# lgw-frank/Short_LDPC_Decoding_OSD

Measured on AMD Instinct MI355X. Metric: decoded frames/sec + FER, (128,64) LDPC NMS-10+OSD-2 @ 2.5 dB, higher is better.
Workload: dtype f32; 1 GPU; nms10_osd2 -- configs[3]: NMS-10 + OSD-2, 2^20 frames over 8 GPUs = 131 072 per GPU; code=CCSDS (128,64), osd_order=2, frames_per_gpu=131072, parallelism=frame-sharded x1, rccl_ranks=1, distinct_batches_per_gpu=4, distinct_frames=524288, bytes_in_plus_out_per_rotation=545783808, nms_kernel=qc16, streams=1, osd_route=front+search

## Files before the change

### short_ldpc_decoding_osd_amd/csrc/ldpc_front.h

```cpp
#pragma once
#include "ldpc_internal.h"
#include "ldpc_wave.h"

namespace ldpc {

struct __attribute__((aligned(16))) FrontLds {
    RankLds rank;
    u64 colbuf[64];
    unsigned mask[4];
    unsigned char pi1[128];
    unsigned char rowsrc[64];
    unsigned char perm[128];
};

struct FrontResult {
    int o1, o2;
    u64 Prow;
    int ns;
};


template <bool GE_LANE_OPAQUE = false>
__device__ __forceinline__ FrontResult front_device_vals(FrontLds &L, unsigned a1, unsigned a2, const u64 *__restrict__ Gcols, int lane)
{
    const float bs = bucket_scale(a1, a2);
    int r1, r2;
    bucket_ranks(L.rank, ((u64)a1 << 32) | (unsigned)(127 - lane), ((u64)a2 << 32) | (unsigned)(63 - lane), bucket_of(a1, bs),
                 bucket_of(a2, bs), lane, r1, r2);
    L.pi1[r1] = (unsigned char)lane;
    L.pi1[r2] = (unsigned char)(lane + 64);
    if (lane < 4) L.mask[lane] = 0;
    wave_fence();
    u64 C1 = Gcols[L.pi1[lane]];
    u64 C2 = Gcols[L.pi1[lane + 64]];
    int rho = lane, idx1 = lane, idx2 = lane + 64;
    int ge_lane = lane;
    if constexpr (GE_LANE_OPAQUE) asm volatile("" : "+v"(ge_lane));
    const int ns = ge_columns(C1, C2, rho, idx1, idx2, ge_lane, nullptr);
    int rankM = lane, rankL = lane;
    if (ns != 0) {
        atomicOr(&L.mask[idx1 >> 5], 1u << (idx1 & 31));
        wave_fence();
        const unsigned m[4] = {L.mask[0], L.mask[1], L.mask[2], L.mask[3]};
        rankM = below_mask(m, idx1);
        rankL = idx2 - below_mask(m, idx2);
    }
    L.perm[rankM] = L.pi1[idx1];
    L.perm[64 + rankL] = L.pi1[idx2];
    L.colbuf[rankL] = C2;
    L.rowsrc[rankM] = (unsigned char)rho;
    wave_fence();
    const u64 R = transpose64(L.colbuf[lane], lane);
    FrontResult res;
    res.Prow = shfl64(R, L.rowsrc[lane]);
    res.o1 = L.perm[lane];
    res.o2 = L.perm[64 + lane];
    res.ns = ns;
    wave_fence();
    return res;
}

template <bool GE_LANE_OPAQUE = false>
__device__ __forceinline__ FrontResult front_device(FrontLds &L, const float *__restrict__ y, long long src,
                                                    const u64 *__restrict__ Gcols, int lane)
{
    return front_device_vals<GE_LANE_OPAQUE>(L, __float_as_uint(y[src * 128 + lane]) & 0x7FFFFFFFu, __float_as_uint(y[src * 128 + 64 + lane]) & 0x7FFFFFFFu, Gcols, lane);
}


}
```

### short_ldpc_decoding_osd_amd/csrc/ldpc_internal.h

```cpp
#pragma once

#include <hip/hip_runtime.h>
#include <stdint.h>

#include <initializer_list>
#include <mutex>
#include <string>
#include <unordered_map>
#include <vector>

#include "../../include/ldpc_osd.h"
#include "ldpc_osd_tables.h"

namespace ldpc {

int fail(int code, const char *fmt, ...) __attribute__((format(printf, 2, 3)));
int hip_fail(hipError_t e, const char *what);

struct NamedPtr {
    const char *name;
    const void *ptr;
};
inline int first_null(const char *who, std::initializer_list<NamedPtr> required)
{
    for (const NamedPtr &r : required)
        if (!r.ptr) return fail(LDPC_E_ARG, "%s: %s is NULL", who, r.name);
    return LDPC_OK;
}

#define LDPC_HIP(call)                                      \
    do {                                                    \
        hipError_t e__ = (call);                            \
        if (e__ != hipSuccess) return ::ldpc::hip_fail(e__, #call); \
    } while (0)

inline unsigned frame_grid(int64_t F) { return (unsigned)(F < 65536 ? F : 65536); }

constexpr int kMaxIters = 64;

struct AlphaArg {
    float a[kMaxIters];
};

struct QcTerm {
    int br, bc, s;
};

}

struct ldpc_code {
    int n = 0, m = 0, k = 0, max_chk_degree = 0, max_var_degree = 0, E = 0;
    std::vector<int32_t> H;
    std::vector<int32_t> G;
    std::vector<int32_t> chk_ptr;
    std::vector<int32_t> chk_var;
    std::vector<int32_t> var_ptr;
    std::vector<int32_t> var_edge;
    bool qc16_ccsds = false;
};

struct ldpc_ctx {
    int device = 0, cu_count = 256;
    ldpc_code code;
    int32_t *d_chk_ptr = nullptr, *d_chk_var = nullptr, *d_var_ptr = nullptr, *d_var_edge = nullptr;
    ldpc::OsdTables osd_tables;
    ldpc::OsdwTables osdw_tables;
    uint64_t *d_Hcols = nullptr;
    uint32_t *d_gen_G = nullptr;
    uint64_t *d_HcolsW = nullptr;
    bool dpp_ror_up = true;
    int dpp_wave_rol_dir = 0;
    bool osd_ok = false;
    bool hosd_ok = false;
    bool hosdx_ok = false;
    bool hosdw_ok = false;
    void *osd_state = nullptr;
    hipEvent_t *timing = nullptr;
    unsigned timing_recorded[LDPC_TIMING_SLOTS] = {};
};

namespace ldpc {

int gf2elim(int32_t *M, int m, int n, std::vector<int32_t> *swaps);
int build_code(ldpc_code &c);
int64_t tep_table(int k, int order, uint8_t *supports, int64_t *boundaries);
int64_t tep_table_fs(int k, int w, uint8_t *supports);
int64_t hosd_pattern_teps(int nseg, const int32_t *bounds, const int32_t *pattern, uint8_t *teps);

int launch_nms(ldpc_ctx *ctx, const float *d_llr, int64_t B, int T, const float *alpha, float w_in, float w_out,
               float *d_soft, float *d_traj, uint64_t *d_hard, uint8_t *d_fail, int kernel, hipStream_t st,
               const int32_t *d_index = nullptr, const int32_t *d_count = nullptr, float *d_rows = nullptr);
int probe_dpp(bool *ror_up, int *wave_rol_dir);
int launch_nms_train(ldpc_ctx *ctx, const float *d_llr, const uint64_t *d_label, int64_t B, int T, const float *alpha,
                     float w_in, float w_out, float *d_loss, float *d_grad, double *d_loss_sum, double *d_grad_sum,
                     float *d_traj, uint64_t *d_hard, uint8_t *d_fail, hipStream_t st);
int check_params(ldpc_ctx *ctx, const ldpc_osd_params *p, bool front_outside, const char *who);
enum class OsdRoute {
    Fused2r,
    Search2r,
    Search2,
    Table,
    Fs,
    PbStaged,
    PbFrontInside,
};
struct OsdPlan {
    OsdRoute route;
    int pb_mode;
};
OsdPlan select_route(const ldpc_ctx *ctx, const ldpc_osd_params *p, bool front_outside);
int osd_launch(ldpc_ctx *ctx, const float *d_y, const int32_t *d_index, const int32_t *d_count, int64_t F, const uint8_t *d_perm,
               const uint64_t *d_parity, const ldpc_osd_params *p, uint64_t *d_cw, float *d_metric, int32_t *d_best, int32_t *d_ntep,
               const uint64_t *d_label, int64_t *d_counts, hipStream_t s, bool *counted);
int eval_and_compact(ldpc_ctx *ctx, const uint64_t *d_hard, const uint64_t *d_label, const uint8_t *d_fail, int64_t B,
                     int64_t *d_counts, int32_t *d_index, int32_t *d_count, hipStream_t st);
int gen_ctx_init(ldpc_ctx *ctx);
void gen_ctx_release(ldpc_ctx *ctx);
int launch_gen(ldpc_ctx *ctx, const ldpc_gen_params *p, int64_t B, float *d_y, uint64_t *d_label_bits, hipStream_t st);

}
```

### short_ldpc_decoding_osd_amd/csrc/ldpc_osd.hip

```cpp
#include <math.h>
#include <stdlib.h>

#include "ldpc_osd_small.h"
#include "ldpc_osd_scan2.h"
#include "ldpc_osd_scan2r.h"
#include "ldpc_osd_fs.h"
#include "ldpc_osd_aux.h"
#include "ldpc_osd_state.h"

namespace ldpc {

int osd_ctx_init(ldpc_ctx *ctx)
{
    const OsdTables &t = ctx->osd_tables;
    ctx->osd_ok = false;
    if (t.n != kOsdN || t.k != kOsdK) return LDPC_OK;
    OsdState *st = new OsdState();
    ctx->osd_state = st;
    {
        int base2[127];
        auto npairs = [](int t) { return (t - 1) / 2 - (t > 63 ? t - 63 : 0) + 1; };
        for (int sidx = 0; sidx < 127; ++sidx) {
            int acc = 0;
            for (int t = sidx + 1; t <= 125; ++t) acc += npairs(t);
            base2[sidx] = acc;
        }
        LDPC_HIP(hipMalloc((void **)&st->d_base2, sizeof(base2)));
        LDPC_HIP(hipMemcpy(st->d_base2, base2, sizeof(base2), hipMemcpyHostToDevice));
    }
    {
        double coef[64], cdf[65], t = 0.5;
        for (int i = 0; i < 64; ++i) coef[i] = (double)(64 - i) / (double)(i + 1);
        for (int q = 0; q < 6; ++q) t = t * t;
        double acc = t;
        cdf[0] = acc;
        for (int i = 0; i < 64; ++i) { t = t * coef[i] * (0.5 / 0.5); acc = acc + t; cdf[i + 1] = acc; }
        LDPC_HIP(hipMalloc((void **)&st->d_cdf_half, sizeof(cdf)));
        LDPC_HIP(hipMemcpy(st->d_cdf_half, cdf, sizeof(cdf), hipMemcpyHostToDevice));
    }
    LDPC_HIP(hipMalloc((void **)&st->d_index_errors, sizeof(unsigned long long)));
    LDPC_HIP(hipMemset(st->d_index_errors, 0, sizeof(unsigned long long)));
    if (int rc = pb_ctx_init(ctx)) return rc;
    ctx->osd_ok = true;
    return LDPC_OK;
}

static void free_stream_ws(StreamWs &w)
{
    (void)hipFree(w.d_perm); (void)hipFree(w.d_parity); (void)hipFree(w.d_index_safe);
    (void)hipFree(w.d_pb_ctl); (void)hipFree(w.d_pb_list); (void)hipFree(w.d_pb_spill); (void)hipFree(w.d_pb_prep);
    (void)hipFree(w.d_pb_carry);
    w = StreamWs();
}

void osd_ctx_release(ldpc_ctx *ctx)
{
    if (OsdState *st = state(ctx)) {
        for (auto &kv : st->ws) free_stream_ws(kv.second);
        (void)hipFree(st->d_base2);
        (void)hipFree(st->d_cdf_half);
        (void)hipFree(st->d_index_errors);
        delete st;
    }
    ctx->osd_state = nullptr;
}

bool stream_capturing(hipStream_t s)
{
    hipStreamCaptureStatus cs = hipStreamCaptureStatusNone;
    return hipStreamIsCapturing(s, &cs) == hipSuccess && cs != hipStreamCaptureStatusNone;
}

static int stream_ws(ldpc_ctx *ctx, hipStream_t s, int64_t frames, StreamWs **out)
{
    OsdState *st = state(ctx);
    std::lock_guard<std::mutex> lock(st->mu);
    StreamWs &w = st->ws[s];
    if (frames > 0 && frames < st->reserve_frames) frames = st->reserve_frames;
    const bool capturing = stream_capturing(s);
    if (frames > w.cap) {
        if (capturing)
            return fail(LDPC_E_NOMEM, "OSD workspace of this stream holds %lld frames, %lld needed: run one call (or "
                        "ldpc_osd_reserve_stream) on the stream before capturing", (long long)w.cap, (long long)frames);
        if (w.captured)
            return fail(LDPC_E_NOMEM, "OSD workspace of this stream (%lld frames) is referenced by a captured graph and cannot grow to "
                        "%lld: destroy the graph and call ldpc_osd_release_stream, or reserve the larger size before capturing",
                        (long long)w.cap, (long long)frames);
        (void)hipFree(w.d_perm); (void)hipFree(w.d_parity);
        w.d_perm = nullptr; w.d_parity = nullptr; w.cap = 0;
        if (hipMalloc((void **)&w.d_perm, (size_t)frames * 128) != hipSuccess ||
            hipMalloc((void **)&w.d_parity, (size_t)frames * 64 * sizeof(u64)) != hipSuccess)
            return fail(LDPC_E_NOMEM, "OSD workspace for %lld frames could not be allocated", (long long)frames);
        w.cap = frames;
    }
    if (capturing) w.captured = true;
    *out = &w;
    return LDPC_OK;
}
static int guarded_index(ldpc_ctx *ctx, const ldpc_osd_params *p, const int32_t *d_index, const int32_t *d_count, int64_t F, hipStream_t s,
                         const int32_t **out)
{
    *out = d_index;
    if (!d_index || p->y_frames <= 0 || F <= 0) return LDPC_OK;
    OsdState *st = state(ctx);
    int *safe;
    {
        std::lock_guard<std::mutex> lock(st->mu);
        StreamWs &w = st->ws[s];
        if (F > w.index_cap) {
            if (stream_capturing(s) || w.captured)
                return fail(LDPC_E_NOMEM, "ldpc_osd_params.y_frames: the checked frame list of this stream holds %lld entries, %lld needed; "
                            "it cannot grow during or after a capture", (long long)w.index_cap, (long long)F);
            (void)hipFree(w.d_index_safe); w.d_index_safe = nullptr; w.index_cap = 0;
            if (hipMalloc((void **)&w.d_index_safe, sizeof(int) * (size_t)F) != hipSuccess)
                return fail(LDPC_E_NOMEM, "checked frame list for %lld frames could not be allocated", (long long)F);
            w.index_cap = F;
        }
        if (stream_capturing(s)) w.captured = true;
        safe = w.d_index_safe;
    }
    const int64_t g = (F + 255) / 256;
    hipLaunchKernelGGL(index_guard_kernel, dim3((unsigned)(g < 1024 ? g : 1024)), dim3(256), 0, s, d_index, d_count, (long long)F,
                       (long long)p->y_frames, safe, st->d_index_errors);
    LDPC_HIP(hipGetLastError());
    *out = safe;
    return LDPC_OK;
}

static unsigned osd_grid(int64_t F)
{
    const int64_t want = (F + 3) / 4;
    return (unsigned)(want < 1 ? 1 : (want < 4096 ? want : 4096));
}


static unsigned grid2r(const ldpc_ctx *ctx, int64_t F) { const int64_t g = (int64_t)ctx->cu_count * 16 * 6; return (unsigned)(F < g ? F : g); }

static void launch_front(ldpc_ctx *ctx, const float *d_y, const int32_t *d_index, const int32_t *d_count, int64_t F, uint8_t *d_perm,
                         u64 *d_parity, int32_t *d_nswaps, hipStream_t s)
{
    hipLaunchKernelGGL(osd_front_kernel, dim3(frame_grid(F)), dim3(64), 0, s, d_y, d_index, d_count, (long long)F,
                       ctx->osd_tables.d_Gcols, d_perm, d_parity, d_nswaps);
}

static int need_osd(const ldpc_ctx *ctx)
{
    return ctx->osd_ok ? LDPC_OK : fail(LDPC_E_UNSUPPORTED, "OSD kernels need an (n=128, k=64) code; this one is (%d,%d)", ctx->code.n, ctx->code.k);
}

static const char *flag_name(unsigned f)
{
    if (f & LDPC_OSD_F_TABLE_SCAN) return "LDPC_OSD_F_TABLE_SCAN";
    if (f & LDPC_OSD_F_PB_BLOCK) return "LDPC_OSD_F_PB_BLOCK";
    if (f & LDPC_OSD_F_PB_REPLAY) return "LDPC_OSD_F_PB_REPLAY";
    if (f & LDPC_OSD_F_READLANE_SCAN) return "LDPC_OSD_F_READLANE_SCAN";
    return "LDPC_OSD_F_PB_FRONT_INSIDE";
}

int check_params(ldpc_ctx *ctx, const ldpc_osd_params *p, bool front_outside, const char *who)
{
    if (int rc = need_osd(ctx)) return rc;
    if (p->order < 0 || p->order > 3) return fail(LDPC_E_ARG, "%s: order %d outside 0..3", who, p->order);
    if (p->algo != LDPC_OSD_CONVENTIONAL && p->algo != LDPC_OSD_FS && p->algo != LDPC_OSD_PB)
        return fail(LDPC_E_ARG, "%s: unknown search algorithm %d", who, p->algo);
    if (p->algo == LDPC_OSD_PB && p->order < 1) return fail(LDPC_E_ARG, "%s: PB-OSD needs order >= 1", who);
    const unsigned f = (unsigned)p->flags;
    const unsigned conv = LDPC_OSD_F_TABLE_SCAN | LDPC_OSD_F_READLANE_SCAN;
    const unsigned pb = LDPC_OSD_F_PB_BLOCK | LDPC_OSD_F_PB_REPLAY | LDPC_OSD_F_PB_FRONT_INSIDE;
    if (f & ~(conv | pb)) return fail(LDPC_E_ARG, "%s: flags 0x%x are no LDPC_OSD_F_* flag", who, f & ~(conv | pb));
    if ((f & conv) && p->algo != LDPC_OSD_CONVENTIONAL)
        return fail(LDPC_E_ARG, "%s: %s needs the conventional algorithm, not %d", who, flag_name(f & conv), p->algo);
    if ((f & LDPC_OSD_F_READLANE_SCAN) && (p->order != 2 || (f & LDPC_OSD_F_TABLE_SCAN)))
        return fail(LDPC_E_ARG, "%s: LDPC_OSD_F_READLANE_SCAN needs order 2 (not %d) and no LDPC_OSD_F_TABLE_SCAN", who, p->order);
    if ((f & pb) && p->algo != LDPC_OSD_PB)
        return fail(LDPC_E_ARG, "%s: %s needs the PB algorithm, not %d", who, flag_name(f & pb), p->algo);
    if ((f & LDPC_OSD_F_PB_REPLAY) && (f & (LDPC_OSD_F_PB_BLOCK | LDPC_OSD_F_PB_FRONT_INSIDE)))
        return fail(LDPC_E_ARG, "%s: LDPC_OSD_F_PB_REPLAY excludes %s", who, flag_name(f & (LDPC_OSD_F_PB_BLOCK | LDPC_OSD_F_PB_FRONT_INSIDE)));
    if ((f & LDPC_OSD_F_PB_FRONT_INSIDE) && front_outside)
        return fail(LDPC_E_ARG, "%s: LDPC_OSD_F_PB_FRONT_INSIDE keeps the front-end results inside the PB kernels, and this call "
                    "supplies or wants them", who);
    return LDPC_OK;
}

OsdPlan select_route(const ldpc_ctx *ctx, const ldpc_osd_params *p, bool front_outside)
{
    const unsigned f = (unsigned)p->flags;
    if (p->algo == LDPC_OSD_FS) return {OsdRoute::Fs, 0};
    if (p->algo == LDPC_OSD_PB)
        return {(f & LDPC_OSD_F_PB_FRONT_INSIDE) ? OsdRoute::PbFrontInside : OsdRoute::PbStaged,
                (f & LDPC_OSD_F_PB_REPLAY) ? 2 : ((f & LDPC_OSD_F_PB_BLOCK) ? 1 : 0)};
    if (p->order != 2 || (f & LDPC_OSD_F_TABLE_SCAN)) return {OsdRoute::Table, 0};
    if ((f & LDPC_OSD_F_READLANE_SCAN) || ctx->dpp_wave_rol_dir == 0) return {OsdRoute::Search2, 0};
    return {front_outside ? OsdRoute::Search2r : OsdRoute::Fused2r, 0};
}

int osd_launch(ldpc_ctx *ctx, const float *d_y, const int32_t *d_index, const int32_t *d_count, int64_t F, const uint8_t *d_perm,
               const uint64_t *d_parity, const ldpc_osd_params *p, uint64_t *d_cw, float *d_metric, int32_t *d_best, int32_t *d_ntep,
               const uint64_t *d_label, int64_t *d_counts, hipStream_t s, bool *counted)
{
    *counted = false;
    const OsdPlan r = select_route(ctx, p, d_perm != nullptr);
    OsdState *st = state(ctx);
    const OsdTables &t = ctx->osd_tables;
    int rc;
    if ((rc = guarded_index(ctx, p, d_index, d_count, F, s, &d_index))) return rc;
    if (!d_perm && r.route != OsdRoute::Fused2r && r.route != OsdRoute::PbFrontInside) {
        StreamWs *w;
        if ((rc = stream_ws(ctx, s, F, &w))) return rc;
        launch_front(ctx, d_y, d_index, d_count, F, w->d_perm, w->d_parity, nullptr, s);
        d_perm = w->d_perm; d_parity = reinterpret_cast<const uint64_t *>(w->d_parity);
    }
    const u64 *const parity = reinterpret_cast<const u64 *>(d_parity);
    u64 *const cw = reinterpret_cast<u64 *>(d_cw);
    const u64 *const label = d_label && d_counts ? reinterpret_cast<const u64 *>(d_label) : nullptr;
    u64 *const counts = label ? reinterpret_cast<u64 *>(d_counts) : nullptr;
    const unsigned g2r = grid2r(ctx, F), g64 = frame_grid(F);
    switch (r.route) {
    case OsdRoute::Fused2r: {
        const auto kernel = ctx->dpp_wave_rol_dir > 0 ? osd_fused2r_kernel<1> : osd_fused2r_kernel<-1>;
        hipLaunchKernelGGL(kernel, dim3(g2r), dim3(64), 0, s, d_y, d_index, d_count, (long long)F, t.d_Gcols, st->d_base2, cw, d_metric,
                           d_best, d_ntep, label, counts);
        *counted = label != nullptr;
        break;
    }
    case OsdRoute::Search2r: {
        const auto kernel = ctx->dpp_wave_rol_dir > 0 ? osd_search2r_kernel<1> : osd_search2r_kernel<-1>;
        hipLaunchKernelGGL(kernel, dim3(g2r), dim3(64), 0, s, d_y, d_index, d_count, (long long)F, d_perm, parity, st->d_base2, cw, d_metric,
                           d_best, d_ntep, label, counts);
        *counted = label != nullptr;
        break;
    }
    case OsdRoute::Search2:
        hipLaunchKernelGGL(osd_search2_kernel, dim3(g64), dim3(64), 0, s, d_y, d_index, d_count, (long long)F, d_perm, parity, st->d_base2,
                           cw, d_metric, d_best, d_ntep);
        break;
    case OsdRoute::Table:
        if (p->order >= 2)
            hipLaunchKernelGGL(osd_search_kernel<1>, dim3(g64), dim3(64), 0, s, d_y, d_index, d_count, (long long)F, d_perm, parity,
                               t.d_tep, (int)t.ntep[p->order], cw, d_metric, d_best, d_ntep);
        else
            hipLaunchKernelGGL(osd_search_kernel<4>, dim3(osd_grid(F)), dim3(256), 0, s, d_y, d_index, d_count, (long long)F, d_perm, parity,
                               t.d_tep, (int)t.ntep[p->order], cw, d_metric, d_best, d_ntep);
        break;
    case OsdRoute::Fs:
        hipLaunchKernelGGL(osd_fs_kernel, dim3(g64), dim3(64), 0, s, d_y, d_index, d_count, (long long)F, d_perm, parity, t.d_tep_fs,
                           fs_params(p, t.n, t.k, t.fs_off, t.fs_cnt), cw, d_metric, d_best, d_ntep);
        break;
    case OsdRoute::PbStaged:
        return launch_pb(ctx, d_y, d_index, d_count, F, d_perm, parity, p, r.pb_mode, false, d_cw, d_metric, d_best, d_ntep, s);
    case OsdRoute::PbFrontInside:
        return launch_pb(ctx, d_y, d_index, d_count, F, nullptr, nullptr, p, r.pb_mode, true, d_cw, d_metric, d_best, d_ntep, s);
    }
    LDPC_HIP(hipGetLastError());
    return LDPC_OK;
}

FsParams fs_params(const ldpc_osd_params *p, int n, int k, const int (&fs_off)[4], const int (&fs_cnt)[4])
{
    FsParams fp;
    fp.order = p->order; fp.quirk = p->fs_reference_quirk != 0;
    fp.beta_term = (float)((double)p->fs_beta * (double)(n - k));
    fp.tau_e = p->fs_tau_e; fp.tau_psc = p->fs_tau_psc;
    for (int w = 0; w < 4; ++w) { fp.cls_off[w] = fs_off[w]; fp.cls_cnt[w] = fs_cnt[w]; }
    return fp;
}

}

using namespace ldpc;

extern "C" {

int ldpc_osd_reserve(ldpc_ctx *ctx, int64_t max_frames)
{
    if (!ctx || max_frames < 0) return fail(LDPC_E_ARG, "ldpc_osd_reserve: bad arguments");
    if (int rc = need_osd(ctx)) return rc;
    {
        OsdState *st = state(ctx);
        std::lock_guard<std::mutex> lock(st->mu);
        if (max_frames > st->reserve_frames) st->reserve_frames = max_frames;
    }
    StreamWs *w;
    return stream_ws(ctx, nullptr, max_frames, &w);
}

int ldpc_osd_reserve_stream(ldpc_ctx *ctx, int64_t max_frames, const ldpc_osd_params *params, void *stream)
{
    if (!ctx || max_frames < 0) return fail(LDPC_E_ARG, "ldpc_osd_reserve_stream: bad arguments");
    int rc;
    if ((rc = need_osd(ctx))) return rc;
    if (params && (rc = check_params(ctx, params, false, "ldpc_osd_reserve_stream"))) return rc;
    StreamWs *w;
    if ((rc = stream_ws(ctx, (hipStream_t)stream, max_frames, &w)) || !params) return rc;
    if (params->algo == LDPC_OSD_PB && max_frames > 0) return pb_reserve(ctx, (hipStream_t)stream, max_frames, params->order);
    return LDPC_OK;
}

int ldpc_osd_release_stream(ldpc_ctx *ctx, void *stream)
{
    if (!ctx) return fail(LDPC_E_ARG, "ldpc_osd_release_stream: null ctx");
    OsdState *st = state(ctx);
    if (!st) return LDPC_OK;
    if (stream_capturing((hipStream_t)stream)) return fail(LDPC_E_ARG, "ldpc_osd_release_stream: the stream is capturing");
    std::lock_guard<std::mutex> lock(st->mu);
    auto it = st->ws.find((hipStream_t)stream);
    if (it != st->ws.end()) { free_stream_ws(it->second); st->ws.erase(it); }
    return LDPC_OK;
}

int ldpc_osd_ge(ldpc_ctx *ctx, const uint64_t *d_rows_in, int64_t F, uint64_t *d_rows_out, uint8_t *d_swaps,
                int32_t *d_nswaps, void *stream)
{
    if (!ctx || F < 0 || (F > 0 && (!d_rows_in || !d_rows_out))) return fail(LDPC_E_ARG, "ldpc_osd_ge: bad arguments");
    if (int rc = need_osd(ctx)) return rc;
    if (F == 0) return LDPC_OK;
    hipLaunchKernelGGL(osd_ge_kernel, dim3(osd_grid(F)), dim3(256), 0, (hipStream_t)stream,
                       reinterpret_cast<const u64 *>(d_rows_in), (long long)F, reinterpret_cast<u64 *>(d_rows_out), d_swaps,
                       d_nswaps);
    LDPC_HIP(hipGetLastError());
    return LDPC_OK;
}

int ldpc_osd_front(ldpc_ctx *ctx, const float *d_y, const int32_t *d_index, const int32_t *d_count, int64_t F,
                   uint8_t *d_perm, uint64_t *d_parity, int32_t *d_nswaps, void *stream)
{
    if (!ctx || F < 0 || (F > 0 && (!d_y || !d_perm || !d_parity))) return fail(LDPC_E_ARG, "ldpc_osd_front: bad arguments");
    if (int rc = need_osd(ctx)) return rc;
    if (F == 0) return LDPC_OK;
    launch_front(ctx, d_y, d_index, d_count, F, d_perm, reinterpret_cast<u64 *>(d_parity), d_nswaps, (hipStream_t)stream);
    LDPC_HIP(hipGetLastError());
    return LDPC_OK;
}

int ldpc_osd_search(ldpc_ctx *ctx, const float *d_y, const int32_t *d_index, const int32_t *d_count, int64_t F,
                    const uint8_t *d_perm, const uint64_t *d_parity, const ldpc_osd_params *p, uint64_t *d_cw,
                    float *d_metric, int32_t *d_best, int32_t *d_ntep, void *stream)
{
    if (!ctx || !p || F < 0 || (F > 0 && (!d_y || !d_cw || !d_perm || !d_parity)))
        return fail(LDPC_E_ARG, "ldpc_osd_search: bad arguments");
    int rc = check_params(ctx, p, true, "ldpc_osd_search");
    if (rc || F == 0) return rc;
    bool counted;
    return osd_launch(ctx, d_y, d_index, d_count, F, d_perm, d_parity, p, d_cw, d_metric, d_best, d_ntep, nullptr, nullptr,
                      (hipStream_t)stream, &counted);
}

int ldpc_osd_decode(ldpc_ctx *ctx, const float *d_y, const int32_t *d_index, const int32_t *d_count, int64_t F,
                    const ldpc_osd_params *p, uint64_t *d_cw, float *d_metric, int32_t *d_best, int32_t *d_ntep,
                    void *stream)
{
    if (!ctx || !p || F < 0 || (F > 0 && (!d_y || !d_cw))) return fail(LDPC_E_ARG, "ldpc_osd_decode: bad arguments");
    int rc = check_params(ctx, p, false, "ldpc_osd_decode");
    if (rc || F == 0) return rc;
    bool counted;
    return osd_launch(ctx, d_y, d_index, d_count, F, nullptr, nullptr, p, d_cw, d_metric, d_best, d_ntep, nullptr, nullptr,
                      (hipStream_t)stream, &counted);
}

int ldpc_osd_index_errors(ldpc_ctx *ctx, int64_t *count)
{
    if (!ctx || !count) return fail(LDPC_E_ARG, "ldpc_osd_index_errors: null argument");
    *count = 0;
    OsdState *st = state(ctx);
    if (!st || !st->d_index_errors) return LDPC_OK;
    unsigned long long v = 0;
    LDPC_HIP(hipMemcpy(&v, st->d_index_errors, sizeof(v), hipMemcpyDeviceToHost));
    *count = (int64_t)v;
    return LDPC_OK;
}

int ldpc_osd_tep_eval(ldpc_ctx *ctx, const float *d_y, const int32_t *d_index, const int32_t *d_count, int64_t F,
                      const uint8_t *d_perm, const uint64_t *d_parity, const uint64_t *d_mask, uint64_t *d_cw, float *d_metric,
                      int32_t *d_hd, void *stream)
{
    if (!ctx || F < 0 || (F > 0 && (!d_y || !d_perm || !d_parity || !d_mask || !d_cw)))
        return fail(LDPC_E_ARG, "ldpc_osd_tep_eval: bad arguments");
    if (int rc = need_osd(ctx)) return rc;
    if (F == 0) return LDPC_OK;
    hipLaunchKernelGGL(osd_tep_eval_kernel, dim3(osd_grid(F)), dim3(256), 0, (hipStream_t)stream, d_y, d_index, d_count, (long long)F,
                       d_perm, reinterpret_cast<const u64 *>(d_parity), reinterpret_cast<const u64 *>(d_mask),
                       reinterpret_cast<u64 *>(d_cw), d_metric, d_hd);
    LDPC_HIP(hipGetLastError());
    return LDPC_OK;
}

int ldpc_osd_counts(ldpc_ctx *ctx, const uint64_t *d_cw, const uint64_t *d_label_bits, const int32_t *d_index,
                    const int32_t *d_count, const int32_t *d_ntep, int64_t F, int64_t *d_counts, void *stream)
{
    if (!ctx || F < 0 || !d_counts || (F > 0 && (!d_cw || !d_label_bits))) return fail(LDPC_E_ARG, "ldpc_osd_counts: bad arguments");
    if (F == 0) return LDPC_OK;
    int64_t g = (F + 1023) / 1024;
    hipLaunchKernelGGL(osd_counts_kernel, dim3((unsigned)(g < 128 ? g : 128)), dim3(256), 0, (hipStream_t)stream,
                       reinterpret_cast<const u64 *>(d_cw), reinterpret_cast<const u64 *>(d_label_bits), d_index, d_count,
                       d_ntep, (long long)F, reinterpret_cast<u64 *>(d_counts));
    LDPC_HIP(hipGetLastError());
    return LDPC_OK;
}

}
```

### short_ldpc_decoding_osd_amd/csrc/ldpc_osd_small.h

```cpp
#pragma once

#include "ldpc_search.h"
#include "ldpc_front.h"

namespace ldpc {

__global__ __launch_bounds__(256) void osd_ge_kernel(const u64 *__restrict__ rows_in, long long F, u64 *__restrict__ rows_out,
        unsigned char *__restrict__ swaps, int *__restrict__ nswaps)
{
    const int lane = threadIdx.x & 63;
    const long long wave = (long long)blockIdx.x * 4 + (threadIdx.x >> 6);
    for (long long f = wave; f < F; f += (long long)gridDim.x * 4) {
        const u64 *src = rows_in + f * 128;
        u64 C1 = transpose64(src[lane * 2], lane);
        u64 C2 = transpose64(src[lane * 2 + 1], lane);
        int rho = lane, idx1 = lane, idx2 = lane + 64;
        const int ns = ge_columns(C1, C2, rho, idx1, idx2, lane, swaps ? swaps + f * 128 : nullptr);
        const u64 R1 = transpose64(C1, lane), R2 = transpose64(C2, lane);
        rows_out[f * 128 + lane * 2] = shfl64(R1, rho);
        rows_out[f * 128 + lane * 2 + 1] = shfl64(R2, rho);
        if (nswaps && lane == 0) nswaps[f] = ns;
    }
}

__global__ __launch_bounds__(64) void osd_front_kernel(const float *__restrict__ y, const int *__restrict__ index, const int *__restrict__ count,
        long long F, const u64 *__restrict__ Gcols, unsigned char *__restrict__ perm_out, u64 *__restrict__ parity_out, int *__restrict__ nswaps)
{
    __shared__ FrontLds L;
    const int lane = threadIdx.x;
    const long long nframes = frame_count(count, F);

    for (long long f = blockIdx.x; f < nframes; f += gridDim.x) {
        const long long src = index ? index[f] : f;
        const FrontResult res = front_device<true>(L, y, src, Gcols, lane);
        perm_out[f * 128 + lane] = (unsigned char)res.o1;
        perm_out[f * 128 + 64 + lane] = (unsigned char)res.o2;
        parity_out[f * 64 + lane] = res.Prow;
        if (nswaps && lane == 0) nswaps[f] = res.ns;
    }
}

template <int WAVES>
__global__ __launch_bounds__(64 * WAVES) void osd_search_kernel(const float *__restrict__ y, const int *__restrict__ index,
        const int *__restrict__ count, long long F, const unsigned char *__restrict__ perm_in, const u64 *__restrict__ parity_in,
        const uchar4 *__restrict__ teps, int ntep, u64 *__restrict__ cw_out, float *__restrict__ metric_out, int *__restrict__ best_out,
        int *__restrict__ ntep_out)
{
    __shared__ SearchLds lds[WAVES];
    const int lane = threadIdx.x & 63;
    SearchLds &L = lds[WAVES == 1 ? 0 : threadIdx.x >> 6];
    const long long nframes = frame_count(count, F);
    const long long wave = (long long)blockIdx.x * WAVES + (threadIdx.x >> 6);

    for (long long f = wave; f < nframes; f += (long long)gridDim.x * WAVES) {
        const long long src = index ? index[f] : f;
        const SearchFrame S = search_prepare(L, y, src, perm_in, parity_in, f, lane);
        float best = __builtin_inff();
        int bestt = 0x7FFFFFFF;
        u64 bestD = 0, bestE = 0;
        float bound = __builtin_inff();
        int trip = 0;
        for (int t0 = 0; t0 < ntep; t0 += 64, ++trip) {
            const int t = t0 + lane;
            if (t < ntep) {
                u64 D, E;
                float mrb, c;
                tep_apply(L, teps[t], S.d0, D, E, mrb);
                if (tep_cost_bounded(L, mrb, D, bound, c) && c < best) { best = c; bestt = t; bestD = D; bestE = E; }
            }
            if ((trip & 7) == 0) bound = wave_min_f32(best);
        }
        wave_argmin(best, bestt, bestD, bestE, lane);
        search_finish(L, S, bestE, bestD, f, lane, cw_out);
        store_results(f, lane, best, bestt, ntep, metric_out, best_out, ntep_out);
    }
}

}
```

Measured before the change: 582.4 million frames/s.

## Prefetch next frame's LLRs and indices, stage Gcols in LDS, shrink front grid

The OSD front kernel now software-pipelines its frame loop. It loads the next frame's received values and the index two frames ahead while the current frame's Gaussian elimination runs, which hides global-load latency. The generator columns are copied once per block into shared memory, so the permuted gathers read LDS instead of global memory. The grid is capped at cu_count*32 blocks so each block loops over several frames and the prefetch has work to overlap. This costs extra registers and LDS per block, and fewer blocks may lower occupancy when the frame count is small.

```diff
diff --git a/short_ldpc_decoding_osd_amd/csrc/ldpc_front.h b/short_ldpc_decoding_osd_amd/csrc/ldpc_front.h
--- a/short_ldpc_decoding_osd_amd/csrc/ldpc_front.h
+++ b/short_ldpc_decoding_osd_amd/csrc/ldpc_front.h
@@ -60,12 +60,4 @@
     return res;
 }
 
-template <bool GE_LANE_OPAQUE = false>
-__device__ __forceinline__ FrontResult front_device(FrontLds &L, const float *__restrict__ y, long long src,
-                                                    const u64 *__restrict__ Gcols, int lane)
-{
-    return front_device_vals<GE_LANE_OPAQUE>(L, __float_as_uint(y[src * 128 + lane]) & 0x7FFFFFFFu, __float_as_uint(y[src * 128 + 64 + lane]) & 0x7FFFFFFFu, Gcols, lane);
 }
-
-
-}
diff --git a/short_ldpc_decoding_osd_amd/csrc/ldpc_internal.h b/short_ldpc_decoding_osd_amd/csrc/ldpc_internal.h
--- a/short_ldpc_decoding_osd_amd/csrc/ldpc_internal.h
+++ b/short_ldpc_decoding_osd_amd/csrc/ldpc_internal.h
@@ -35,6 +35,13 @@
     } while (0)
 
 inline unsigned frame_grid(int64_t F) { return (unsigned)(F < 65536 ? F : 65536); }
+
+constexpr int kFrontGridX = 1;
+inline unsigned front_grid(int cu_count, int64_t F)
+{
+    const int64_t g = (int64_t)cu_count * 32 * kFrontGridX;
+    return (unsigned)(F < g ? F : g);
+}
 
 constexpr int kMaxIters = 64;
 
diff --git a/short_ldpc_decoding_osd_amd/csrc/ldpc_osd.hip b/short_ldpc_decoding_osd_amd/csrc/ldpc_osd.hip
--- a/short_ldpc_decoding_osd_amd/csrc/ldpc_osd.hip
+++ b/short_ldpc_decoding_osd_amd/csrc/ldpc_osd.hip
@@ -139,7 +139,7 @@
 static void launch_front(ldpc_ctx *ctx, const float *d_y, const int32_t *d_index, const int32_t *d_count, int64_t F, uint8_t *d_perm,
                          u64 *d_parity, int32_t *d_nswaps, hipStream_t s)
 {
-    hipLaunchKernelGGL(osd_front_kernel, dim3(frame_grid(F)), dim3(64), 0, s, d_y, d_index, d_count, (long long)F,
+    hipLaunchKernelGGL(osd_front_kernel, dim3(front_grid(ctx->cu_count, F)), dim3(64), 0, s, d_y, d_index, d_count, (long long)F,
                        ctx->osd_tables.d_Gcols, d_perm, d_parity, d_nswaps);
 }
 
diff --git a/short_ldpc_decoding_osd_amd/csrc/ldpc_osd_small.h b/short_ldpc_decoding_osd_amd/csrc/ldpc_osd_small.h
--- a/short_ldpc_decoding_osd_amd/csrc/ldpc_osd_small.h
+++ b/short_ldpc_decoding_osd_amd/csrc/ldpc_osd_small.h
@@ -27,16 +27,37 @@
         long long F, const u64 *__restrict__ Gcols, unsigned char *__restrict__ perm_out, u64 *__restrict__ parity_out, int *__restrict__ nswaps)
 {
     __shared__ FrontLds L;
+    __shared__ u64 Gl[128];
     const int lane = threadIdx.x;
+    const u64 g1 = Gcols[lane], g2 = Gcols[64 + lane];
     const long long nframes = frame_count(count, F);
-
-    for (long long f = blockIdx.x; f < nframes; f += gridDim.x) {
-        const long long src = index ? index[f] : f;
-        const FrontResult res = front_device<true>(L, y, src, Gcols, lane);
-        perm_out[f * 128 + lane] = (unsigned char)res.o1;
-        perm_out[f * 128 + 64 + lane] = (unsigned char)res.o2;
-        parity_out[f * 64 + lane] = res.Prow;
-        if (nswaps && lane == 0) nswaps[f] = res.ns;
+    const long long G = gridDim.x;
+    long long f0 = blockIdx.x, f1 = f0 + G, f2 = f1 + G;
+    int ia = 0, ib = 0;
+    unsigned a1 = 0, a2 = 0;
+    if (index && f0 < nframes) ia = index[f0];
+    if (index && f1 < nframes) ib = index[f1];
+    if (f0 < nframes) {
+        const long long src = index ? (long long)ia : f0;
+        a1 = __float_as_uint(y[src * 128 + lane]) & 0x7FFFFFFFu; a2 = __float_as_uint(y[src * 128 + 64 + lane]) & 0x7FFFFFFFu;
+    }
+    Gl[lane] = g1; Gl[64 + lane] = g2;
+    while (f0 < nframes) {
+        unsigned yb1 = 0, yb2 = 0;
+        if (f1 < nframes) {
+            const long long src = index ? (long long)ib : f1;
+            yb1 = __float_as_uint(y[src * 128 + lane]); yb2 = __float_as_uint(y[src * 128 + 64 + lane]);
+        }
+        int ic = 0;
+        if (index && f2 < nframes) ic = index[f2];
+        const FrontResult res = front_device_vals<true>(L, a1, a2, Gl, lane);
+        perm_out[f0 * 128 + lane] = (unsigned char)res.o1;
+        perm_out[f0 * 128 + 64 + lane] = (unsigned char)res.o2;
+        parity_out[f0 * 64 + lane] = res.Prow;
+        if (nswaps && lane == 0) nswaps[f0] = res.ns;
+        f0 = f1; f1 = f2; f2 += G;
+        asm volatile("" : "+v"(yb1), "+v"(yb2));
+        ib = ic; a1 = yb1 & 0x7FFFFFFFu; a2 = yb2 & 0x7FFFFFFFu;
     }
 }
 
```

New measurement: 593.8 million frames/s, median of 6. 2.0% higher.
